# siyi-wind/MDViT

Hardware: AMD Instinct MI355X
Metric: 512x512 images/sec MDViT train step (fwd+bwd, two-sweep, AdamW) (higher is better)
Workload: dtype bf16x3 (fp32 storage; GEMM operands split hi+lo bf16, fp32 accumulate); 1 GPU; MDViT Sup+MLPFM train step, 4 domain(s) x bs=4 per GPU, 512x512, drop_rate=0.1 drop_path=0.1, bf16x3 GEMMs, data-parallel x1

## Files before the change

mdvit_amd/csrc/attn.hip:

```cpp
#include "common.h"
#include "conv_tile.h"

namespace {

constexpr int FA_T = 64;

struct FaGeom {
    int B, H, W, N, C, heads, Ch, s3, s5, s7;
    float scale;
};

typedef float fap_f32x16 __attribute__((ext_vector_type(16)));

template <int CH, bool SOFTMAX>
__global__ __launch_bounds__(256) void fa_partial_kernel(const float* __restrict__ X, long ldx, const float* __restrict__ Y, long ldy,
                                                         const float* __restrict__ ysc, float yscale,
                                                         float* __restrict__ ws_m, float* __restrict__ ws_s, float* __restrict__ ws_P,
                                                         FaGeom g, int NT, int NSUB,
                                                         const float* __restrict__ outp = nullptr, float* __restrict__ dU = nullptr, float* __restrict__ e_part = nullptr) {
    constexpr int GW = CH < 32 ? 32 : CH, NB = (GW + 31) / 32, GQ = GW / 4;
    constexpr int STAGE = 2 * FA_T * GW, RED = 4 * NB * 32 * NB * 32;
    __shared__ __attribute__((aligned(16))) float sm[(STAGE > RED ? STAGE : RED) + 3 * NB * 32 + (SOFTMAX ? 2 * 256 : 0)];
    float* xs = sm;
    float* ys = sm + FA_T * GW;
// ... 394 lines not shown
    }
}

__global__ __launch_bounds__(256) void fa_bwd_prep_kernel(const float* __restrict__ dout, const float* __restrict__ qkv,
                                                          const float* __restrict__ out, const float* __restrict__ a,
                                                          float* __restrict__ dU, float* __restrict__ e, FaGeom g) {
    extern __shared__ float s_e[];
    const int b = blockIdx.y, C = g.C, QC = C >> 2;
    for (int i = threadIdx.x; i < C; i += blockDim.x) s_e[i] = 0.f;
    __syncthreads();
    const long T = (long)gridDim.x * blockDim.x;
    const long t0 = (long)blockIdx.x * blockDim.x + threadIdx.x;
    const int c = (int)(t0 % QC) * 4;
    float4 av = make_float4(1.f, 1.f, 1.f, 1.f);
    if (a) av = *reinterpret_cast<const float4*>(a + (long)b * C + c);
    float4 acc = make_float4(0.f, 0.f, 0.f, 0.f);
    const long total = (long)g.N * QC;
    for (long i = t0; i < total; i += T) {
        const long tok = (long)b * g.N + i / QC;
        const float4 G = *reinterpret_cast<const float4*>(dout + tok * C + c);
        const float4 q = *reinterpret_cast<const float4*>(qkv + tok * 3 * C + c);
        if (dU) *reinterpret_cast<float4*>(dU + tok * C + c) = make_float4(av.x * G.x * q.x, av.y * G.y * q.y, av.z * G.z * q.z, av.w * G.w * q.w);
        if (e) {
            const float4 o = *reinterpret_cast<const float4*>(out + tok * C + c);
            acc.x = fmaf(G.x, o.x, acc.x); acc.y = fmaf(G.y, o.y, acc.y); acc.z = fmaf(G.z, o.z, acc.z); acc.w = fmaf(G.w, o.w, acc.w);
        }
    }
    if (e) {
        atomicAdd(&s_e[c], acc.x); atomicAdd(&s_e[c + 1], acc.y); atomicAdd(&s_e[c + 2], acc.z); atomicAdd(&s_e[c + 3], acc.w);
        __syncthreads();
        for (int i = threadIdx.x; i < C; i += blockDim.x) e[((long)b * gridDim.x + blockIdx.x) * C + i] = s_e[i];
    }
}

typedef float fa_f32x16 __attribute__((ext_vector_type(16)));
template <int CH>
__global__ __launch_bounds__(256) __attribute__((amdgpu_waves_per_eu(2, 2))) void fa_bwd_apply_tab_kernel(const float* __restrict__ dout, const float* __restrict__ qkv,
                                                               const float* __restrict__ U, const float* __restrict__ dVc,
                                                               const float* __restrict__ Mmat, const float* __restrict__ a,
                                                               const float* __restrict__ kmax, const float* __restrict__ ksum,
                                                               const float* __restrict__ dMp, int NTS,
                                                               float* __restrict__ dqkv, FaGeom g, int tokens_per_block) {
    constexpr int C = 8 * CH, C3 = 3 * C, LPT = C / 4, SLOTS = 256 / LPT, LPH = CH / 4, L4 = CH / 4, NS = 8 * L4 + CH;
    __shared__ __attribute__((aligned(16))) float sM[C * CH], sD[C * CH];
    __shared__ __attribute__((aligned(16))) float4 tab[NS][LPT];
    __shared__ float s_tc[C];
    const int b = blockIdx.y;
    for (int i = threadIdx.x; i < C * CH; i += 256) {
        sM[i] = Mmat[(long)b * C * CH + i];
        float dm = 0.f;
        const float* pp = dMp + ((long)b * NTS) * C * CH + i;
        const long rs = (long)C * CH;
        for (int t0 = 0; t0 < NTS; t0 += 8) {
            float v8[8];
#pragma unroll
            for (int u = 0; u < 8; ++u) { const int t = t0 + u; v8[u] = pp[(long)(t < NTS ? t : NTS - 1) * rs]; if (t >= NTS) v8[u] = 0.f; }
#pragma unroll
            for (int u = 0; u < 8; ++u) dm += v8[u];
        }
        sD[i] = dm;
    }
    __syncthreads();
    if (threadIdx.x < C) {
        float tc = 0.f;
#pragma unroll
        for (int e = 0; e < CH; ++e) tc = fmaf(sD[threadIdx.x * CH + e], sM[threadIdx.x * CH + e], tc);
        s_tc[threadIdx.x] = tc;
    }
    for (int i = threadIdx.x; i < NS * LPT; i += 256) {
        const int slot = i / LPT, qq = i % LPT, hl = qq % LPH, hb = (qq / LPH) * CH, cc0 = 4 * qq;
        float4 v;
        if (slot < 8 * L4) {
            const int sl = slot % (4 * L4);
            const float* src = (slot < 4 * L4 ? sM : sD) + (cc0 + sl / L4) * CH + 4 * (hl ^ (sl % L4));
            v = *reinterpret_cast<const float4*>(src);
        } else {
            const int l = slot - 8 * L4, e = 4 * (hl ^ (l >> 2)) + (l & 3);
            v = *reinterpret_cast<const float4*>(sD + (hb + e) * CH + 4 * hl);
        }
        tab[slot][qq] = v;
    }
    __syncthreads();
    const int q = threadIdx.x % LPT, slot = threadIdx.x / LPT;
    const int c0 = 4 * q;
    const long ci = (long)b * C + c0;
    const float4 a4 = a ? *reinterpret_cast<const float4*>(a + ci) : make_float4(1.f, 1.f, 1.f, 1.f);
    const float4 km4 = *reinterpret_cast<const float4*>(kmax + ci);
    float4 is4 = *reinterpret_cast<const float4*>(ksum + ci);
    is4 = make_float4(1.0f / is4.x, 1.0f / is4.y, 1.0f / is4.z, 1.0f / is4.w);
    const float4 tc4 = *reinterpret_cast<const float4*>(s_tc + c0);
    const float inv_scale = 1.0f / g.scale;
    const int n_beg = blockIdx.x * tokens_per_block, n_end = min(g.N, n_beg + tokens_per_block);
    struct Rows { float4 g, k, v, u, c; };
    auto request = [&](Rows& r, int n) __attribute__((always_inline)) {
        const long tok = (long)b * g.N + min(n, g.N - 1);
        r.g = *reinterpret_cast<const float4*>(dout + tok * C + c0);
        r.k = *reinterpret_cast<const float4*>(qkv + tok * C3 + C + c0);
        r.v = *reinterpret_cast<const float4*>(qkv + tok * C3 + 2 * C + c0);
        r.u = *reinterpret_cast<const float4*>(U + tok * C + c0);
        r.c = *reinterpret_cast<const float4*>(dVc + tok * C + c0);
    };
    auto compute = [&](const Rows& r, int n) __attribute__((always_inline)) {
        float dfa[CH], vv[CH], pp[CH];
        dfa[0] = g.scale * a4.x * r.g.x; dfa[1] = g.scale * a4.y * r.g.y; dfa[2] = g.scale * a4.z * r.g.z; dfa[3] = g.scale * a4.w * r.g.w;
        vv[0] = r.v.x; vv[1] = r.v.y; vv[2] = r.v.z; vv[3] = r.v.w;
        pp[0] = expf(r.k.x - km4.x) * is4.x; pp[1] = expf(r.k.y - km4.y) * is4.y; pp[2] = expf(r.k.z - km4.z) * is4.z; pp[3] = expf(r.k.w - km4.w) * is4.w;
#pragma unroll
        for (int j = 0; j < 4; ++j) {
            dfa[4 + j] = fa_dpp_quad_xor<1>(dfa[j]); vv[4 + j] = fa_dpp_quad_xor<1>(vv[j]); pp[4 + j] = fa_dpp_quad_xor<1>(pp[j]);
            if constexpr (CH == 16) {
                dfa[8 + j] = fa_dpp_quad_xor<2>(dfa[j]); dfa[12 + j] = fa_dpp_quad_xor<3>(dfa[j]);
                vv[8 + j] = fa_dpp_quad_xor<2>(vv[j]); vv[12 + j] = fa_dpp_quad_xor<3>(vv[j]);
                pp[8 + j] = fa_dpp_quad_xor<2>(pp[j]); pp[12 + j] = fa_dpp_quad_xor<3>(pp[j]);
            }
        }
        float dq[4], dk[4], dv[4] = {0.f, 0.f, 0.f, 0.f};
        const float uu[4] = {r.u.x, r.u.y, r.u.z, r.u.w}, cc[4] = {r.c.x, r.c.y, r.c.z, r.c.w}, tcv[4] = {tc4.x, tc4.y, tc4.z, tc4.w};
        asm volatile("" ::: "memory");
#pragma unroll
        for (int j = 0; j < 4; ++j) {
            float s1 = 0.f, s2 = 0.f;
#pragma unroll
            for (int l4 = 0; l4 < L4; ++l4) {
                const float4 m4 = tab[L4 * j + l4][q], d4 = tab[4 * L4 + L4 * j + l4][q];
                s1 = fmaf(dfa[4 * l4 + 0], m4.x, s1); s1 = fmaf(dfa[4 * l4 + 1], m4.y, s1); s1 = fmaf(dfa[4 * l4 + 2], m4.z, s1); s1 = fmaf(dfa[4 * l4 + 3], m4.w, s1);
                s2 = fmaf(vv[4 * l4 + 0], d4.x, s2); s2 = fmaf(vv[4 * l4 + 1], d4.y, s2); s2 = fmaf(vv[4 * l4 + 2], d4.z, s2); s2 = fmaf(vv[4 * l4 + 3], d4.w, s2);
            }
            dq[j] = fmaf(dfa[j] * inv_scale, uu[j], s1);
            dk[j] = pp[j] * (s2 - tcv[j]);
        }
#pragma unroll
        for (int l = 0; l < CH; ++l) {
            const float4 dc = tab[8 * L4 + l][q];
            dv[0] = fmaf(pp[l], dc.x, dv[0]); dv[1] = fmaf(pp[l], dc.y, dv[1]); dv[2] = fmaf(pp[l], dc.z, dv[2]); dv[3] = fmaf(pp[l], dc.w, dv[3]);
        }
        if (n < n_end) {
            float* drow = dqkv + ((long)b * g.N + n) * C3 + c0;
            *reinterpret_cast<float4*>(drow) = make_float4(dq[0], dq[1], dq[2], dq[3]);
            *reinterpret_cast<float4*>(drow + C) = make_float4(dk[0], dk[1], dk[2], dk[3]);
            *reinterpret_cast<float4*>(drow + 2 * C) = make_float4(dv[0] + cc[0], dv[1] + cc[1], dv[2] + cc[2], dv[3] + cc[3]);
        }
    };
    Rows ra, rb;
    int n = n_beg + slot;
    request(ra, n);
    for (; n < n_end; n += 2 * SLOTS) {
        request(rb, n + SLOTS);
        compute(ra, n);
        request(ra, n + 2 * SLOTS);
        compute(rb, n + SLOTS);
    }
}

template <int CH, int ROLE>
__device__ __forceinline__ void fa_apply3_tiles(const float* __restrict__ dout, const float* __restrict__ qkv, const float* __restrict__ U, const float* __restrict__ dVc,
                                                float* __restrict__ dqkv, const FaGeom& g, const float* sKV, const float* sD, const float* s_a, const float* s_km,
                                                const float* s_ks, const float* s_tc, int b, int g0, int slot, int tiles_per_block, int bx) {
    constexpr int GW = CH, NB = (GW + 31) / 32, NQ = GW / 8, KS = GW / 2, LD = GW + 1;
    const int C = g.C, C3 = 3 * C;
    const int lane = threadIdx.x & 63;
    const int t = lane & 31, half = lane >> 5;
    const int ntiles = (g.N + 31) / 32;
    const int tile_beg = bx * tiles_per_block, tile_end = min(ntiles, tile_beg + tiles_per_block);
    const float inv_scale = 1.0f / g.scale;
    struct Rows { float4 a[NQ], b[NQ]; };
    auto request = [&](Rows& r, int tile) __attribute__((always_inline)) {
        const long tok = (long)b * g.N + min(tile * 32 + t, g.N - 1);
        const float* arow = ROLE == 0 ? dout + tok * C + g0 : qkv + tok * C3 + C + g0;
        const float* brow = ROLE == 0 ? U + tok * C + g0 : (ROLE == 1 ? qkv + tok * C3 + 2 * C + g0 : dVc + tok * C + g0);
#pragma unroll
        for (int q = 0; q < NQ; ++q) {
            const int cq = 32 * (q / 4) + 8 * (q % 4) + 4 * half;
            r.a[q] = *reinterpret_cast<const float4*>(arow + cq);
            r.b[q] = *reinterpret_cast<const float4*>(brow + cq);
        }
    };
    auto compute = [&](const Rows& r, int tile) __attribute__((always_inline)) {
        const int n = tile * 32 + t;
        const bool ok = n < g.N;
        const float z = ok ? 1.f : 0.f;
        const long tok = (long)b * g.N + (ok ? n : g.N - 1);
        float xo[NQ][4], el[NQ][4];
#pragma unroll
        for (int q = 0; q < NQ; ++q) {
            const int cq = 32 * (q / 4) + 8 * (q % 4) + 4 * half;
            const float4 a4 = r.a[q], b4 = r.b[q];
            if (ROLE == 0) {
                const float4 s4 = *reinterpret_cast<const float4*>(s_a + cq);
                xo[q][0] = z * g.scale * s4.x * a4.x; xo[q][1] = z * g.scale * s4.y * a4.y;
                xo[q][2] = z * g.scale * s4.z * a4.z; xo[q][3] = z * g.scale * s4.w * a4.w;
                el[q][0] = b4.x; el[q][1] = b4.y; el[q][2] = b4.z; el[q][3] = b4.w;
            } else {
                const float4 m4 = *reinterpret_cast<const float4*>(s_km + cq);
                const float4 i4 = *reinterpret_cast<const float4*>(s_ks + cq);
                const float p0 = z * expf(a4.x - m4.x) * i4.x, p1 = z * expf(a4.y - m4.y) * i4.y;
                const float p2 = z * expf(a4.z - m4.z) * i4.z, p3 = z * expf(a4.w - m4.w) * i4.w;
                if (ROLE == 1) {
                    xo[q][0] = z * b4.x; xo[q][1] = z * b4.y; xo[q][2] = z * b4.z; xo[q][3] = z * b4.w;
                    el[q][0] = p0; el[q][1] = p1; el[q][2] = p2; el[q][3] = p3;
                } else {
                    xo[q][0] = p0; xo[q][1] = p1; xo[q][2] = p2; xo[q][3] = p3;
                    el[q][0] = b4.x; el[q][1] = b4.y; el[q][2] = b4.z; el[q][3] = b4.w;
                }
            }
        }
        fa_f32x16 acc[NB];
#pragma unroll
        for (int ob = 0; ob < NB; ++ob)
#pragma unroll
            for (int rr = 0; rr < 16; ++rr) acc[ob][rr] = 0.f;
        asm volatile("" ::: "memory");
#pragma unroll
        for (int ob = 0; ob < NB; ++ob) {
            const int orow = 32 * ob + t;
            const bool rok = orow < GW;
            const int orc = rok ? orow : 0;
#pragma unroll
            for (int kk = 0; kk < KS; ++kk) {
                const int q = kk / 4, j = kk % 4;
                const int kc = 32 * (q / 4) + 8 * (q % 4) + 4 * half + j;
                float w = ROLE == 0 ? sKV[orc * LD + kc] : (ROLE == 1 ? sD[orc * LD + kc] : sD[kc * LD + orc]);
                if (!rok) w = 0.f;
                acc[ob] = __builtin_amdgcn_mfma_f32_32x32x2f32(w, xo[q][j], acc[ob], 0, 0, 0);
            }
        }
        if (ok) {
            float* drow = dqkv + tok * C3 + ROLE * C + g0;
#pragma unroll
            for (int q = 0; q < NQ; ++q) {
                const int ob = q / 4, r0 = 4 * (q % 4);
                const int cq = 32 * (q / 4) + 8 * (q % 4) + 4 * half;
                float4 d;
                if (ROLE == 0) {
                    d.x = fmaf(xo[q][0] * inv_scale, el[q][0], acc[ob][r0 + 0]); d.y = fmaf(xo[q][1] * inv_scale, el[q][1], acc[ob][r0 + 1]);
                    d.z = fmaf(xo[q][2] * inv_scale, el[q][2], acc[ob][r0 + 2]); d.w = fmaf(xo[q][3] * inv_scale, el[q][3], acc[ob][r0 + 3]);
                } else if (ROLE == 1) {
                    const float4 t4 = *reinterpret_cast<const float4*>(s_tc + cq);
                    d.x = el[q][0] * (acc[ob][r0 + 0] - t4.x); d.y = el[q][1] * (acc[ob][r0 + 1] - t4.y);
                    d.z = el[q][2] * (acc[ob][r0 + 2] - t4.z); d.w = el[q][3] * (acc[ob][r0 + 3] - t4.w);
                } else {
                    d.x = acc[ob][r0 + 0] + el[q][0]; d.y = acc[ob][r0 + 1] + el[q][1];
                    d.z = acc[ob][r0 + 2] + el[q][2]; d.w = acc[ob][r0 + 3] + el[q][3];
                }
                *reinterpret_cast<float4*>(drow + cq) = d;
            }
        }
    };
    Rows ra, rb;
    int tile = tile_beg + slot;
    if (tile < tile_end) request(ra, tile);
    for (; tile < tile_end; tile += 4) {
        request(rb, min(tile + 2, ntiles - 1));
        compute(ra, tile);
        if (tile + 2 < tile_end) {
            request(ra, min(tile + 4, ntiles - 1));
            compute(rb, tile + 2);
        }
    }
}

template <int CH>
__global__ __launch_bounds__(384) __attribute__((amdgpu_waves_per_eu(CH >= 64 ? 2 : 3, CH >= 64 ? 2 : 3))) void fa_bwd_apply3_kernel(const float* __restrict__ dout, const float* __restrict__ qkv,
                                                           const float* __restrict__ U, const float* __restrict__ dVc,
                                                           const float* __restrict__ Mmat, const float* __restrict__ a,
                                                           const float* __restrict__ kmax, const float* __restrict__ ksum,
                                                           const float* __restrict__ dMp, int NTS,
                                                           float* __restrict__ dqkv, FaGeom g, int tiles_per_block, int gx, int xcd_map) {
    static_assert(CH >= 32 && CH % 8 == 0, "one head per channel group");
    constexpr int GW = CH, NB = (GW + 31) / 32, NQ = GW / 8, KS = GW / 2, LD = GW + 1, NTH = 384;
    __shared__ float sKV[GW * LD], sD[GW * LD];
    __shared__ __attribute__((aligned(16))) float s_a[GW], s_km[GW], s_ks[GW], s_tc[GW];
    const int C = g.C, C3 = 3 * C;
    int bx, by, bz;
    if (xcd_map) {
        const int nwg = gridDim.x, heads = C / GW;
        const int i = blockIdx.x, slot = (i & 7) * (nwg >> 3) + (i >> 3);
        by = slot % heads; bx = (slot / heads) % gx; bz = slot / (heads * gx);
    } else { bx = blockIdx.x; by = blockIdx.y; bz = blockIdx.z; }
    const int b = bz, g0 = by * GW;
    for (int i = threadIdx.x; i < GW * GW; i += NTH) {
        const int r = i / GW, cc = i % GW;
        sKV[r * LD + cc] = Mmat[((long)b * C + g0 + r) * CH + cc];
        float dm = 0.f;
        const float* pp = dMp + (((long)b * NTS) * C + g0 + r) * CH + cc;
        const long rs = (long)C * CH;
        for (int t0 = 0; t0 < NTS; t0 += 8) {
            float v8[8];
#pragma unroll
            for (int u = 0; u < 8; ++u) { const int t = t0 + u; v8[u] = pp[(long)(t < NTS ? t : NTS - 1) * rs]; if (t >= NTS) v8[u] = 0.f; }
#pragma unroll
            for (int u = 0; u < 8; ++u) dm += v8[u];
        }
        sD[r * LD + cc] = dm;
    }
    for (int i = threadIdx.x; i < GW; i += NTH) {
        const long ci = (long)b * C + g0 + i;
        s_a[i] = a ? a[ci] : 1.f; s_km[i] = kmax[ci]; s_ks[i] = 1.0f / ksum[ci];
    }
    __syncthreads();
    for (int i = threadIdx.x; i < GW; i += NTH) {
        float tc = 0.f;
        for (int e = 0; e < CH; ++e) tc = fmaf(sD[i * LD + e], sKV[i * LD + e], tc);
        s_tc[i] = tc;
    }
    __syncthreads();
    const int wave = threadIdx.x >> 6;
    const int role = wave % 3, slot = wave / 3;
    if (role == 0) fa_apply3_tiles<CH, 0>(dout, qkv, U, dVc, dqkv, g, sKV, sD, s_a, s_km, s_ks, s_tc, b, g0, slot, tiles_per_block, bx);
    else if (role == 1) fa_apply3_tiles<CH, 1>(dout, qkv, U, dVc, dqkv, g, sKV, sD, s_a, s_km, s_ks, s_tc, b, g0, slot, tiles_per_block, bx);
    else fa_apply3_tiles<CH, 2>(dout, qkv, U, dVc, dqkv, g, sKV, sD, s_a, s_km, s_ks, s_tc, b, g0, slot, tiles_per_block, bx);
}

__device__ __forceinline__ void da_fwd_body(float* sm, const float* __restrict__ label, const float* __restrict__ W1, const float* __restrict__ b1,
                                            const float* __restrict__ W2, const float* __restrict__ b2, float* __restrict__ a, int D, int hid, int C, int heads) {
    float* h1 = sm;
    float* z = sm + hid;
    float* zpart = z + C;
    const int b = blockIdx.x, Ch = C / heads, BD = blockDim.x;
    for (int i = threadIdx.x; i < hid; i += BD) {
        float s = 0.f;
        for (int d = 0; d < D; ++d) s = fmaf(label[(long)b * D + d], W1[(long)i * D + d], s);
        h1[i] = fmaxf(s + b1[i], 0.f);
    }
    __syncthreads();
    const bool vec = (hid & 3) == 0 && (reinterpret_cast<uintptr_t>(W2) & 15) == 0;
    const int nq = vec ? hid >> 2 : hid;
    int G = BD / C;
    if (G < 1) G = 1;
    if (G > nq) G = nq;
    for (int c0 = 0; c0 < C; c0 += BD / G) {
        const int c = c0 + (int)threadIdx.x / G, seg = (int)threadIdx.x % G;
        if (c < C && (int)threadIdx.x < (BD / G) * G) {
            const int u0 = (int)((long)nq * seg / G), u1 = (int)((long)nq * (seg + 1) / G);
            const float* wr = W2 + (long)c * hid;
            float s = 0.f;
            if (vec) {
                int u = u0;
                for (; u + 8 <= u1; u += 8) {
                    float4 w4[8];
#pragma unroll
                    for (int q = 0; q < 8; ++q) w4[q] = *reinterpret_cast<const float4*>(wr + 4 * (u + q));
#pragma unroll
                    for (int q = 0; q < 8; ++q) {
                        const int i = 4 * (u + q);
                        s = fmaf(h1[i], w4[q].x, s); s = fmaf(h1[i + 1], w4[q].y, s); s = fmaf(h1[i + 2], w4[q].z, s); s = fmaf(h1[i + 3], w4[q].w, s);
                    }
                }
                for (; u < u1; ++u) {
                    const float4 w4 = *reinterpret_cast<const float4*>(wr + 4 * u);
                    const int i = 4 * u;
                    s = fmaf(h1[i], w4.x, s); s = fmaf(h1[i + 1], w4.y, s); s = fmaf(h1[i + 2], w4.z, s); s = fmaf(h1[i + 3], w4.w, s);
                }
            } else {
                for (int i = u0; i < u1; ++i) s = fmaf(h1[i], wr[i], s);
            }
            zpart[seg * C + c] = s;
        }
    }
    __syncthreads();
    for (int c = threadIdx.x; c < C; c += BD) {
        float s = zpart[c];
        for (int g = 1; g < G; ++g) s += zpart[g * C + c];
        z[c] = s + b2[c];
    }
    __syncthreads();
    for (int c = threadIdx.x; c < C; c += BD) {
        const int ch = c % Ch;
        float m = -INFINITY;
        for (int hh = 0; hh < heads; ++hh) m = fmaxf(m, z[hh * Ch + ch]);
        float s = 0.f;
        for (int hh = 0; hh < heads; ++hh) s += expf(z[hh * Ch + ch] - m);
        a[(long)b * C + c] = expf(z[c] - m) / s;
    }
}
__global__ __launch_bounds__(1024) void da_fwd_kernel(const float* __restrict__ label, const float* __restrict__ W1, const float* __restrict__ b1,
                                                      const float* __restrict__ W2, const float* __restrict__ b2, float* __restrict__ a,
                                                      int D, int hid, int C, int heads) {
    extern __shared__ float sm[];
    da_fwd_body(sm, label, W1, b1, W2, b2, a, D, hid, C, heads);
}
__global__ __launch_bounds__(1024) void da_fwd_many_kernel(MdvitDaMany m, const float* __restrict__ label, int D) {
    extern __shared__ float sm[];
    const int i = blockIdx.y;
    da_fwd_body(sm, label, m.W1[i], m.b1[i], m.W2[i], m.b2[i], m.a[i], D, m.hid[i], m.C[i], m.heads[i]);
}

__device__ __forceinline__ void da_bwd_stage1_body(float* sm, const float* __restrict__ label, const float* __restrict__ W1, const float* __restrict__ b1,
                                                   const float* __restrict__ W2, const float* __restrict__ a, const float* __restrict__ e,
                                                   float* __restrict__ dzbuf, float* __restrict__ hbuf, float* __restrict__ dhbuf,
                                                   int D, int hid, int C, int heads, float scale) {
    float* dz = sm;
    const int b = blockIdx.x, Ch = C / heads;
    for (int c = threadIdx.x; c < C; c += blockDim.x) {
        const int ch = c % Ch;
        float tot = 0.f;
        for (int hh = 0; hh < heads; ++hh) tot += e[(long)b * C + hh * Ch + ch];
        const float v = scale * (e[(long)b * C + c] - a[(long)b * C + c] * tot);
        dz[c] = v;
        dzbuf[(long)b * C + c] = v;
    }
    __syncthreads();
    float* tpart = sm + C;
    const int BD = blockDim.x;
    const int nseg = hid <= BD ? BD / hid : 1;
    for (int i0 = 0; i0 < hid; i0 += BD) {
        const int i = i0 + (int)threadIdx.x % (hid <= BD ? hid : BD), seg = hid <= BD ? (int)threadIdx.x / hid : 0;
        if (i < hid && seg < nseg) {
            const int c_beg = (int)((long)C * seg / nseg), c_end = (int)((long)C * (seg + 1) / nseg);
            float t = 0.f;
#pragma unroll 4
            for (int c = c_beg; c < c_end; ++c) t = fmaf(dz[c], W2[(long)c * hid + i], t);
            tpart[seg * hid + i] = t;
        }
    }
    __syncthreads();
    for (int i = threadIdx.x; i < hid; i += blockDim.x) {
        float s = 0.f;
        for (int d = 0; d < D; ++d) s = fmaf(label[(long)b * D + d], W1[(long)i * D + d], s);
        const float h = s + b1[i];
        float t = 0.f;
        for (int seg = 0; seg < nseg; ++seg) t += tpart[seg * hid + i];
        hbuf[(long)b * hid + i] = fmaxf(h, 0.f);
        dhbuf[(long)b * hid + i] = h > 0.f ? t : 0.f;
    }
}
__global__ __launch_bounds__(1024) void da_bwd_stage1_kernel(const float* __restrict__ label, const float* __restrict__ W1, const float* __restrict__ b1,
                                                            const float* __restrict__ W2, const float* __restrict__ a, const float* __restrict__ e,
                                                            float* __restrict__ dzbuf, float* __restrict__ hbuf, float* __restrict__ dhbuf,
                                                            int D, int hid, int C, int heads, float scale) {
    extern __shared__ float sm[];
    da_bwd_stage1_body(sm, label, W1, b1, W2, a, e, dzbuf, hbuf, dhbuf, D, hid, C, heads, scale);
}
__device__ __forceinline__ void da_bwd_stage2_body(const float* __restrict__ label, const float* __restrict__ dzbuf,
                                                   const float* __restrict__ hbuf, const float* __restrict__ dhbuf,
                                                   float* __restrict__ dW1, float* __restrict__ db1, float* __restrict__ dW2, float* __restrict__ db2,
                                                   int B, int D, int hid, int C) {
    const long i = (long)blockIdx.x * blockDim.x + threadIdx.x;
    const long nW2 = (long)C * hid, nW1 = (long)hid * D;
    if (i < nW2) {
        const int c = (int)(i / hid), j = (int)(i % hid);
        float s = 0.f;
        for (int b = 0; b < B; ++b) s = fmaf(dzbuf[(long)b * C + c], hbuf[(long)b * hid + j], s);
        dW2[i] = s;
    } else if (i < nW2 + nW1) {
        const long k = i - nW2;
        const int j = (int)(k / D), d = (int)(k % D);
        float s = 0.f;
        for (int b = 0; b < B; ++b) s = fmaf(dhbuf[(long)b * hid + j], label[(long)b * D + d], s);
        dW1[k] = s;
    } else if (i < nW2 + nW1 + C) {
        const int c = (int)(i - nW2 - nW1);
        float s = 0.f;
        for (int b = 0; b < B; ++b) s += dzbuf[(long)b * C + c];
        db2[c] = s;
    } else if (i < nW2 + nW1 + C + hid) {
        const int j = (int)(i - nW2 - nW1 - C);
        float s = 0.f;
        for (int b = 0; b < B; ++b) s += dhbuf[(long)b * hid + j];
        db1[j] = s;
    }
}
__global__ __launch_bounds__(256) void da_bwd_stage2_kernel(const float* __restrict__ label, const float* __restrict__ dzbuf,
                                                            const float* __restrict__ hbuf, const float* __restrict__ dhbuf,
                                                            float* __restrict__ dW1, float* __restrict__ db1, float* __restrict__ dW2, float* __restrict__ db2,
                                                            int B, int D, int hid, int C) {
    da_bwd_stage2_body(label, dzbuf, hbuf, dhbuf, dW1, db1, dW2, db2, B, D, hid, C);
}
__device__ __forceinline__ long da_many_ws_offset(const MdvitDaMany& m, int i, int B) {
    long off = 0;
    for (int j = 0; j < i; ++j) off += (long)B * m.C[j] + 2L * B * m.hid[j];
    return off;
}
__global__ __launch_bounds__(1024) void da_bwd_many_stage1_kernel(MdvitDaMany m, MdvitDaManyGrads g, const float* __restrict__ label, float* __restrict__ ws, int B, int D,
                                                                 float scale) {
    extern __shared__ float sm[];
    const int i = blockIdx.y;
    if (!g.e[i]) return;
    float* dzbuf = ws + da_many_ws_offset(m, i, B);
    float* hbuf = dzbuf + (long)B * m.C[i];
    float* dhbuf = hbuf + (long)B * m.hid[i];
    da_bwd_stage1_body(sm, label, m.W1[i], m.b1[i], m.W2[i], m.a[i], g.e[i], dzbuf, hbuf, dhbuf, D, m.hid[i], m.C[i], m.heads[i], scale);
}
__global__ __launch_bounds__(256) void da_bwd_many_stage2_kernel(MdvitDaMany m, MdvitDaManyGrads g, const float* __restrict__ label, const float* __restrict__ ws, int B, int D) {
    const int i = blockIdx.y;
    const int hid = m.hid[i], C = m.C[i];
    if (!g.e[i] || (long)blockIdx.x * blockDim.x >= (long)C * hid + (long)hid * D + C + hid) return;
    const float* dzbuf = ws + da_many_ws_offset(m, i, B);
    const float* hbuf = dzbuf + (long)B * C;
    const float* dhbuf = hbuf + (long)B * hid;
    da_bwd_stage2_body(label, dzbuf, hbuf, dhbuf, g.dW1[i], g.db1[i], g.dW2[i], g.db2[i], B, D, hid, C);
}

bool make_geom(FaGeom& g, int B, int H, int W, int C, int heads, int s3, int s5, int s7) {
    if (B <= 0 || H <= 0 || W <= 0 || C <= 0 || heads <= 0 || C % heads != 0 || C % 4 != 0) return false;
    if (s3 + s5 + s7 != heads) return false;
    g.B = B; g.H = H; g.W = W; g.N = H * W; g.C = C; g.heads = heads; g.Ch = C / heads; g.s3 = s3; g.s5 = s5; g.s7 = s7;
    g.scale = 1.0f / sqrtf((float)g.Ch);
    return true;
}

size_t fa_ws_floats(int B, int N, int C, int heads) {
    const int Ch = C / heads;
    const long NT = (N + FA_T - 1) / FA_T;
    const long fwd = (long)B * NT * C * (2 + Ch);
    const long wg_rows = (long)(cdiv(C, 32) + 2) * B > 1024 ? (long)(cdiv(C, 32) + 2) * B : 1024;
    const long part = wg_rows * 32 * 50 > 1024L * B * C ? wg_rows * 32 * 50 : 1024L * B * C;
    const long bwd = 2L * B * N * C + (long)B * C * (1 + Ch) + (long)B * NT * C * Ch + part;
    return (size_t)(fwd > bwd ? fwd : bwd);
}

int fa_nsub(int NT) { return NT >= 128 ? 8 : (NT >= 64 ? 4 : (NT >= 16 ? 2 : 1)); }

bool fa_built(const FaGeom& g) { return ((g.Ch == 8 || g.Ch == 16) && g.heads == 8) || ((g.Ch == 40 || g.Ch == 64) && g.C <= 512); }
#define FA_CHECK_BUILT(fn, g) MDVIT_CHECK_ARG(fa_built(g), MDVIT_E_SHAPE, fn ": C=%d with %d heads (head dim %d) not built: built are 8 heads at C = 64 / 128 (head dim 8 / 16) " \
                                              "and head dim 40 / 64 with C <= 512 (8 heads at C = 320 / 512)", (g).C, (g).heads, (g).Ch)

int quad_grid(long work_quads, int QC, int max_blocks) {
    int a = QC, b = 256;
    while (b) { int t = a % b; a = b; b = t; }
    const int gmul = QC / a;
    long want = (work_quads + 256L * 4 - 1) / (256L * 4);
    if (want > max_blocks) want = max_blocks;
    if (want < 1) want = 1;
    return (int)((want + gmul - 1) / gmul * gmul);
}

}

extern "C" size_t mdvit_factoratt_ws_bytes(int32_t B, int32_t N, int32_t C, int32_t heads) {
    if (B <= 0 || N <= 0 || C <= 0 || heads <= 0 || C % heads) return 0;
    return fa_ws_floats(B, N, C, heads) * sizeof(float);
}

extern "C" int mdvit_factoratt_fwd(const float* qkv, const float* w3, const float* b3, const float* w5, const float* b5,
                                   const float* w7, const float* b7, const float* a, float* out, float* U, float* kmax, float* ksum, float* Mmat,
                                   void* ws, size_t ws_bytes, int32_t B, int32_t H, int32_t W, int32_t C, int32_t heads,
                                   int32_t s3, int32_t s5, int32_t s7, void* stream) {
    hipStream_t s = (hipStream_t)stream;
    FaGeom g;
    MDVIT_CHECK_ARG(make_geom(g, B, H, W, C, heads, s3, s5, s7), MDVIT_E_SHAPE, "factoratt_fwd: bad geometry B=%d H=%d W=%d C=%d heads=%d splits=%d/%d/%d", B, H, W, C, heads, s3, s5, s7);
    FA_CHECK_BUILT("factoratt_fwd", g);
    MDVIT_CHECK_ARG(ws_bytes >= fa_ws_floats(B, g.N, C, heads) * sizeof(float), MDVIT_E_WORKSPACE, "factoratt_fwd: workspace too small (%zu bytes)", ws_bytes);
    const int Ch = g.Ch, NT0 = cdiv(g.N, FA_T);
    const int NSUB = fa_nsub(NT0);
    const int NT = cdiv(NT0, NSUB);
    float* ws_m = (float*)ws;
    float* ws_s = ws_m + (long)B * NT * C;
    float* ws_P = ws_s + (long)B * NT * C;
#define FA_PART_STREAM(CHV) fa_partial_stream_launch<CHV, true>(dim3(NT, 1, B), s, qkv + C, (long)3 * C, qkv + 2 * C, (long)3 * C, nullptr, 1.f, ws_m, ws_s, ws_P, g, NT0, NSUB, nullptr, nullptr, nullptr)
#define FA_PART_TILES(CHV) hipLaunchKernelGGL((fa_partial_kernel<CHV, true>), dim3(NT, C / CHV, B), dim3(256), 0, s, \
                       qkv + C, (long)3 * C, qkv + 2 * C, (long)3 * C, (const float*)nullptr, 1.f, ws_m, ws_s, ws_P, g, NT0, NSUB)
    switch (Ch) {
        case 8: FA_PART_STREAM(8); break;
        case 16: FA_PART_STREAM(16); break;
        case 40: FA_PART_TILES(40); break;
        case 64: FA_PART_TILES(64); break;
    }
#undef FA_PART_STREAM
#undef FA_PART_TILES
    if (NT > 8)
        hipLaunchKernelGGL((fa_combine_softmax_kernel<32>), dim3(cdiv((long)C * g.Ch, 8), B), dim3(256), 0, s, ws_m, ws_s, ws_P, kmax, ksum, Mmat, g, NT);
    else if (NT > 2)
        hipLaunchKernelGGL((fa_combine_softmax_kernel<4>), dim3(cdiv((long)C * g.Ch, 64), B), dim3(256), 0, s, ws_m, ws_s, ws_P, kmax, ksum, Mmat, g, NT);
    else
        hipLaunchKernelGGL((fa_combine_softmax_kernel<1>), dim3(cdiv((long)C * g.Ch, 256), B), dim3(256), 0, s, ws_m, ws_s, ws_P, kmax, ksum, Mmat, g, NT);
    const int c5 = s3 * Ch, c7 = (s3 + s5) * Ch;
    const CtGeom cg{B, g.H, g.W};
    {
        const int xoff[3] = {2 * C, 2 * C + c5, 2 * C + c7}, yoff[3] = {0, c5, c7}, ncls[3] = {s3 * Ch, s5 * Ch, s7 * Ch};
        const float* const ws3[3] = {w3, w5, w7};
        const float* const bs3[3] = {b3, b5, b7};
        launch_conv3<false>(qkv, 3L * C, xoff, ws3, bs3, U, (long)C, yoff, cg, ncls, s);
    }
    {
        const int TLN = max(1, 256 / C), block = TLN * C;
        int tpb = TLN * 32;
        while (tpb > TLN * 8 && (long)cdiv(g.N, tpb) * B < 1024) tpb /= 2;
        while ((long)cdiv(g.N, tpb) * B > 8192) tpb *= 2;
        dim3 grid(cdiv(g.N, tpb), B);
#define FA_OUT_LAUNCH(CHV) hipLaunchKernelGGL((fa_out_kernel<CHV>), grid, dim3(block), sizeof(float) * FA_OUT_U * TLN * C, s, qkv, U, Mmat, a, out, g, TLN, tpb)
        switch (Ch) {
            case 8: FA_OUT_LAUNCH(8); break;
            case 16: FA_OUT_LAUNCH(16); break;
            case 40: FA_OUT_LAUNCH(40); break;
            case 64: FA_OUT_LAUNCH(64); break;
        }
#undef FA_OUT_LAUNCH
    }
    MDVIT_LAUNCH_CHECK();
    return MDVIT_OK;
}

extern "C" int mdvit_factoratt_bwd(const float* dout, const float* qkv, const float* out, const float* U,
                                   const float* w3, const float* b3, const float* w5, const float* b5, const float* w7, const float* b7,
                                   const float* a, const float* kmax, const float* ksum, const float* Mmat,
                                   float* dqkv, float* e, float* dw3, float* db3, float* dw5, float* db5, float* dw7, float* db7,
                                   void* ws, size_t ws_bytes, int32_t B, int32_t H, int32_t W, int32_t C, int32_t heads,
                                   int32_t s3, int32_t s5, int32_t s7, void* stream) {
    hipStream_t s = (hipStream_t)stream;
    FaGeom g;
    MDVIT_CHECK_ARG(make_geom(g, B, H, W, C, heads, s3, s5, s7), MDVIT_E_SHAPE, "factoratt_bwd: bad geometry B=%d H=%d W=%d C=%d heads=%d", B, H, W, C, heads);
    FA_CHECK_BUILT("factoratt_bwd", g);
    MDVIT_CHECK_ARG(ws_bytes >= fa_ws_floats(B, g.N, C, heads) * sizeof(float), MDVIT_E_WORKSPACE, "factoratt_bwd: workspace too small (%zu bytes)", ws_bytes);
    MDVIT_CHECK_ARG((a == nullptr) == (e == nullptr), MDVIT_E_SHAPE, "factoratt_bwd: a and e must both be given or both be NULL");
    const int Ch = g.Ch, NT = cdiv(g.N, FA_T);
    float* dU = (float*)ws;
    float* dVc = dU + (long)B * g.N * C;
    float* tcol = dVc + (long)B * g.N * C;
    float* dM = tcol + (long)B * C;
    float* ws_P = dM + (long)B * C * Ch;
    const bool want_wgrad = dw3 != nullptr;
    MDVIT_CHECK_ARG(want_wgrad ? (db3 && dw5 && db5 && dw7 && db7) : !(db3 || dw5 || db5 || dw7 || db7), MDVIT_E_SHAPE,
                    "factoratt_bwd: the six crpe gradient outputs must be all given or all NULL");
    if (dqkv == nullptr) {
        MDVIT_CHECK_ARG(e != nullptr && !want_wgrad, MDVIT_E_SHAPE, "factoratt_bwd: dqkv == NULL asks for e alone");
        const int QC0 = C / 4;
        const int gx = quad_grid((long)g.N * QC0, QC0, 512);
        float* e_part = ws_P + (long)B * NT * C * Ch;
        hipLaunchKernelGGL(fa_bwd_prep_kernel, dim3(gx, B), dim3(256), sizeof(float) * C, s, dout, qkv, out, a, (float*)nullptr, e_part, g);
        MDVIT_LAUNCH_CHECK();
        return mdvit_reduce_partials_batched(e_part, B, gx, C, e, s);
    }
    const int NSUBb = fa_nsub(NT), NTS = cdiv(NT, NSUBb);
    float* e_part = ws_P + (long)B * NT * C * Ch;
#define FA_PART_STREAM(CHV) fa_partial_stream_launch<CHV, false>(dim3(NTS, 1, B), s, qkv, (long)3 * C, dout, (long)C, a, g.scale, nullptr, nullptr, ws_P, g, NT, NSUBb, out, dU, e ? e_part : nullptr)
#define FA_PART_TILES(CHV) hipLaunchKernelGGL((fa_partial_kernel<CHV, false>), dim3(NTS, C / CHV, B), dim3(256), 0, s, \
                       qkv, (long)3 * C, dout, (long)C, a, g.scale, (float*)nullptr, (float*)nullptr, ws_P, g, NT, NSUBb, out, dU, e ? e_part : (float*)nullptr)
    switch (Ch) {
        case 8: FA_PART_STREAM(8); break;
        case 16: FA_PART_STREAM(16); break;
        case 40: FA_PART_TILES(40); break;
        case 64: FA_PART_TILES(64); break;
    }
#undef FA_PART_STREAM
#undef FA_PART_TILES
    if (e) {
        const int rc = mdvit_reduce_partials_batched(e_part, B, NTS, C, e, s);
        if (rc != MDVIT_OK) return rc;
    }
    const int c5 = s3 * Ch, c7 = (s3 + s5) * Ch;
    const CtGeom cg{B, g.H, g.W};
    if (want_wgrad) {
        float* wg_part = ws_P + (long)B * NT * C * Ch;
        const int goff[3] = {0, c5, c7}, xoff3[3] = {2 * C, 2 * C + c5, 2 * C + c7}, ncls3[3] = {s3 * Ch, s5 * Ch, s7 * Ch};
        float* const dws[3] = {dw3, dw5, dw7};
        float* const dbs[3] = {db3, db5, db7};
        launch_conv3_wgrad(dU, (long)C, goff, qkv, 3L * C, xoff3, dws, dbs, wg_part, cg, ncls3, s, 0);
    }
    {
        const int off[3] = {0, c5, c7}, ncls[3] = {s3 * Ch, s5 * Ch, s7 * Ch};
        const float* const ws3[3] = {w3, w5, w7};
        launch_conv3<true>(dU, (long)C, off, ws3, nullptr, dVc, (long)C, off, cg, ncls, s);
    }
    if (Ch >= 32) {
        const int ntiles = cdiv(g.N, 32);
        int tpb = 8;
        while (tpb > 2 && (long)cdiv(ntiles, tpb) * heads * B < 256) tpb /= 2;
        const int gx = cdiv(ntiles, tpb);
        const long nwg = (long)gx * heads * B;
        const int xcd_map = nwg % 8 == 0 && nwg < (1L << 30);
        dim3 grid = xcd_map ? dim3((unsigned)nwg, 1, 1) : dim3(gx, heads, B);
        if (Ch == 40) hipLaunchKernelGGL((fa_bwd_apply3_kernel<40>), grid, dim3(384), 0, s, dout, qkv, U, dVc, Mmat, a, kmax, ksum, ws_P, NTS, dqkv, g, tpb, gx, xcd_map);
        else hipLaunchKernelGGL((fa_bwd_apply3_kernel<64>), grid, dim3(384), 0, s, dout, qkv, U, dVc, Mmat, a, kmax, ksum, ws_P, NTS, dqkv, g, tpb, gx, xcd_map);
    } else {
        int tpbk = Ch == 8 ? 1024 : 512;
        while (tpbk > 128 && (long)cdiv(g.N, tpbk) * B < 512) tpbk /= 2;
        const dim3 grid(cdiv(g.N, tpbk), B);
        if (Ch == 8) hipLaunchKernelGGL(fa_bwd_apply_tab_kernel<8>, grid, dim3(256), 0, s, dout, qkv, U, dVc, Mmat, a, kmax, ksum, ws_P, NTS, dqkv, g, tpbk);
        else hipLaunchKernelGGL(fa_bwd_apply_tab_kernel<16>, grid, dim3(256), 0, s, dout, qkv, U, dVc, Mmat, a, kmax, ksum, ws_P, NTS, dqkv, g, tpbk);
    }
    MDVIT_LAUNCH_CHECK();
    return MDVIT_OK;
}

extern "C" int mdvit_factoratt_wgrad(const float* qkv, void* ws, size_t ws_bytes, float* dw3, float* db3, float* dw5, float* db5,
                                     float* dw7, float* db7, int32_t B, int32_t H, int32_t W, int32_t C, int32_t heads,
                                     int32_t s3, int32_t s5, int32_t s7, int32_t accumulate, void* stream) {
    hipStream_t s = (hipStream_t)stream;
    FaGeom g;
    MDVIT_CHECK_ARG(make_geom(g, B, H, W, C, heads, s3, s5, s7), MDVIT_E_SHAPE, "factoratt_wgrad: bad geometry");
    MDVIT_CHECK_ARG(ws_bytes >= fa_ws_floats(B, g.N, C, heads) * sizeof(float), MDVIT_E_WORKSPACE, "factoratt_wgrad: workspace too small");
    MDVIT_CHECK_ARG(dw3 && db3 && dw5 && db5 && dw7 && db7, MDVIT_E_SHAPE, "factoratt_wgrad: all six outputs are required");
    const int Ch = g.Ch, NT = cdiv(g.N, FA_T);
    const float* dU = (const float*)ws;
    float* wg_part = (float*)ws + 2L * B * g.N * C + (long)B * C * (1 + Ch) + (long)B * NT * C * Ch;
    const int c5 = s3 * Ch, c7 = (s3 + s5) * Ch;
    const CtGeom cg{B, g.H, g.W};
    const int goff[3] = {0, c5, c7}, xoff3[3] = {2 * C, 2 * C + c5, 2 * C + c7}, ncls3[3] = {s3 * Ch, s5 * Ch, s7 * Ch};
    float* const dws[3] = {dw3, dw5, dw7};
    float* const dbs[3] = {db3, db5, db7};
    launch_conv3_wgrad(dU, (long)C, goff, qkv, 3L * C, xoff3, dws, dbs, wg_part, cg, ncls3, s, accumulate);
    MDVIT_LAUNCH_CHECK();
    return MDVIT_OK;
}

extern "C" int mdvit_da_fwd(const float* label, const float* W1, const float* b1, const float* W2, const float* b2, float* a,
                            int32_t B, int32_t D, int32_t hid, int32_t C, int32_t heads, void* stream) {
    MDVIT_CHECK_ARG(B > 0 && D > 0 && hid > 0 && C > 0 && heads > 0 && C % heads == 0, MDVIT_E_SHAPE, "da_fwd: bad shape");
    const int G = max(1, min(1024 / C, hid));
    hipLaunchKernelGGL(da_fwd_kernel, dim3(B), dim3(1024), sizeof(float) * (hid + C + (size_t)(G + 1) * C), (hipStream_t)stream, label, W1, b1, W2, b2, a, D, hid, C, heads);
    MDVIT_LAUNCH_CHECK();
    return MDVIT_OK;
}

extern "C" int mdvit_da_fwd_many(const MdvitDaMany* m, const float* label, int32_t B, int32_t D, void* stream) {
    MDVIT_CHECK_ARG(m && label && B > 0 && D > 0 && m->n > 0 && m->n <= MDVIT_DA_MANY_MAX, MDVIT_E_SHAPE, "da_fwd_many: bad arguments");
    size_t smem = 0;
    for (int i = 0; i < m->n; ++i) {
        const int C = m->C[i], hid = m->hid[i];
        MDVIT_CHECK_ARG(m->W1[i] && m->b1[i] && m->W2[i] && m->b2[i] && m->a[i] && hid > 0 && C > 0 && m->heads[i] > 0 && C % m->heads[i] == 0, MDVIT_E_SHAPE,
                        "da_fwd_many: bad adapter %d", i);
        const int G = max(1, min(1024 / C, hid));
        smem = std::max(smem, sizeof(float) * (hid + C + (size_t)(G + 1) * C));
    }
    MDVIT_CHECK_ARG(smem <= 64 * 1024, MDVIT_E_SHAPE, "da_fwd_many: an adapter needs %zu bytes of LDS", smem);
    hipLaunchKernelGGL(da_fwd_many_kernel, dim3(B, m->n), dim3(1024), smem, (hipStream_t)stream, *m, label, D);
    MDVIT_LAUNCH_CHECK();
    return MDVIT_OK;
}

extern "C" size_t mdvit_da_ws_bytes(int32_t B, int32_t hid, int32_t C) {
    if (B <= 0 || hid <= 0 || C <= 0) return 0;
    return sizeof(float) * ((size_t)B * C + 2 * (size_t)B * hid);
}

extern "C" size_t mdvit_da_many_ws_bytes(const MdvitDaMany* m, int32_t B) {
    if (!m || m->n <= 0 || m->n > MDVIT_DA_MANY_MAX || B <= 0) return 0;
    size_t t = 0;
    for (int i = 0; i < m->n; ++i) t += mdvit_da_ws_bytes(B, m->hid[i], m->C[i]);
    return t;
}

extern "C" int mdvit_da_bwd_many(const MdvitDaMany* m, const MdvitDaManyGrads* g, const float* label, float scale, void* ws, size_t ws_bytes, int32_t B, int32_t D,
                                 void* stream) {
    MDVIT_CHECK_ARG(m && g && m->n > 0 && m->n <= MDVIT_DA_MANY_MAX && B > 0 && D > 0, MDVIT_E_SHAPE, "da_bwd_many: bad shape");
    MDVIT_CHECK_ARG(ws_bytes >= mdvit_da_many_ws_bytes(m, B), MDVIT_E_WORKSPACE, "da_bwd_many: workspace too small");
    size_t smem = 0;
    long most = 0;
    bool any = false;
    for (int i = 0; i < m->n; ++i) {
        MDVIT_CHECK_ARG(m->hid[i] > 0 && m->C[i] > 0 && m->heads[i] > 0 && m->C[i] % m->heads[i] == 0, MDVIT_E_SHAPE, "da_bwd_many: bad adapter shape");
        if (!g->e[i]) continue;
        MDVIT_CHECK_ARG(g->dW1[i] && g->db1[i] && g->dW2[i] && g->db2[i], MDVIT_E_SHAPE, "da_bwd_many: an adapter with e needs its four gradient outputs");
        any = true;
        smem = max(smem, sizeof(float) * (m->C[i] + (size_t)max(m->hid[i], 1024)));
        most = max(most, (long)m->C[i] * m->hid[i] + (long)m->hid[i] * D + m->C[i] + m->hid[i]);
    }
    if (!any) return MDVIT_OK;
    hipStream_t s = (hipStream_t)stream;
    hipLaunchKernelGGL(da_bwd_many_stage1_kernel, dim3(B, m->n), dim3(1024), smem, s, *m, *g, label, (float*)ws, B, D, scale);
    hipLaunchKernelGGL(da_bwd_many_stage2_kernel, dim3(cdiv(most, 256), m->n), dim3(256), 0, s, *m, *g, label, (const float*)ws, B, D);
    MDVIT_LAUNCH_CHECK();
    return MDVIT_OK;
}

extern "C" int mdvit_da_bwd(const float* label, const float* W1, const float* b1, const float* W2, const float* b2, const float* a,
                            const float* e, float scale, float* dW1, float* db1, float* dW2, float* db2, void* ws, size_t ws_bytes,
// ... 15 lines not shown
```

Before: 527.1 images/s.

## Coalesce factor-attention apply loads/stores via per-wave LDS transpose staging

Result: no change. 529.1 images/s (median of 6 runs) (+0.4%).

```diff
diff --git a/mdvit_amd/csrc/attn.hip b/mdvit_amd/csrc/attn.hip
--- a/mdvit_amd/csrc/attn.hip
+++ b/mdvit_amd/csrc/attn.hip
@@ -570,56 +570,70 @@
     }
 }
 
+__device__ __forceinline__ void fa_wave_lds_sync() {
+    __builtin_amdgcn_fence(__ATOMIC_RELEASE, "wavefront");
+    __builtin_amdgcn_wave_barrier();
+    __builtin_amdgcn_fence(__ATOMIC_ACQUIRE, "wavefront");
+}
+typedef float fa_f4 __attribute__((ext_vector_type(4)));
 template <int CH, int ROLE>
 __device__ __forceinline__ void fa_apply3_tiles(const float* __restrict__ dout, const float* __restrict__ qkv, const float* __restrict__ U, const float* __restrict__ dVc,
                                                 float* __restrict__ dqkv, const FaGeom& g, const float* sKV, const float* sD, const float* s_a, const float* s_km,
-                                                const float* s_ks, const float* s_tc, int b, int g0, int slot, int tiles_per_block, int bx) {
-    constexpr int GW = CH, NB = (GW + 31) / 32, NQ = GW / 8, KS = GW / 2, LD = GW + 1;
+                                                const float* s_ks, const float* s_tc, float* stg, int b, int g0, int slot, int tiles_per_block, int bx) {
+    constexpr int GW = CH, NB = (GW + 31) / 32, NQ = GW / 8, KS = GW / 2, LD = GW + 1, QR = GW / 4, LDR = GW + 4;
+    static_assert(32 * QR == 64 * NQ && (LDR / 4) % 2 == 1, "NQ wave-wide fa_f4 instructions cover the 32 x GW tile; odd slot stride");
     const int C = g.C, C3 = 3 * C;
     const int lane = threadIdx.x & 63;
     const int t = lane & 31, half = lane >> 5;
     const int ntiles = (g.N + 31) / 32;
     const int tile_beg = bx * tiles_per_block, tile_end = min(ntiles, tile_beg + tiles_per_block);
     const float inv_scale = 1.0f / g.scale;
-    struct Rows { float4 a[NQ], b[NQ]; };
-    auto request = [&](Rows& r, int tile) __attribute__((always_inline)) {
-        const long tok = (long)b * g.N + min(tile * 32 + t, g.N - 1);
-        const float* arow = ROLE == 0 ? dout + tok * C + g0 : qkv + tok * C3 + C + g0;
-        const float* brow = ROLE == 0 ? U + tok * C + g0 : (ROLE == 1 ? qkv + tok * C3 + 2 * C + g0 : dVc + tok * C + g0);
-#pragma unroll
-        for (int q = 0; q < NQ; ++q) {
-            const int cq = 32 * (q / 4) + 8 * (q % 4) + 4 * half;
-            r.a[q] = *reinterpret_cast<const float4*>(arow + cq);
-            r.b[q] = *reinterpret_cast<const float4*>(brow + cq);
+    const float* xbase = (ROLE == 0 ? dout + g0 : (ROLE == 1 ? qkv + 2 * C + g0 : qkv + C + g0)) + (long)b * g.N * (ROLE == 0 ? C : C3);
+    const float* ebase = (ROLE == 0 ? U + g0 : (ROLE == 1 ? qkv + C + g0 : dVc + g0)) + (long)b * g.N * (ROLE == 1 ? C3 : C);
+    float* dbase = dqkv + (long)b * g.N * C3 + ROLE * C + g0;
+    const unsigned ldx = ROLE == 0 ? C : C3, lde = ROLE == 1 ? C3 : C;
+    auto request = [&](fa_f4 (&r)[NQ], const float* base, unsigned ld, int tile) __attribute__((always_inline)) {
+#pragma unroll
+        for (int v = 0; v < NQ; ++v) {
+            const int i = lane + 64 * v, row = i / QR, qd = i % QR;
+            const unsigned tr = (unsigned)min(tile * 32 + row, g.N - 1);
+            r[v] = *reinterpret_cast<const fa_f4*>(reinterpret_cast<const char*>(base) + 4u * (tr * ld + 4u * qd));
         }
     };
-    auto compute = [&](const Rows& r, int tile) __attribute__((always_inline)) {
+    auto transpose = [&](const fa_f4 (&r)[NQ], fa_f4 (&tq)[NQ]) __attribute__((always_inline)) {
+        fa_wave_lds_sync();
+#pragma unroll
+        for (int v = 0; v < NQ; ++v) { const int i = lane + 64 * v; *reinterpret_cast<fa_f4*>(stg + (i / QR) * LDR + 4 * (i % QR)) = r[v]; }
+        fa_wave_lds_sync();
+#pragma unroll
+        for (int q = 0; q < NQ; ++q) tq[q] = *reinterpret_cast<const fa_f4*>(stg + t * LDR + 32 * (q / 4) + 8 * (q % 4) + 4 * half);
+    };
+    auto softmax_p = [&](const fa_f4 k4, int cq, float z, float (&p)[4]) __attribute__((always_inline)) {
+        const fa_f4 m4 = *reinterpret_cast<const fa_f4*>(s_km + cq);
+        const fa_f4 i4 = *reinterpret_cast<const fa_f4*>(s_ks + cq);
+        p[0] = z * expf(k4.x - m4.x) * i4.x; p[1] = z * expf(k4.y - m4.y) * i4.y;
+        p[2] = z * expf(k4.z - m4.z) * i4.z; p[3] = z * expf(k4.w - m4.w) * i4.w;
+    };
+    auto compute = [&](const fa_f4 (&xr)[NQ], int tile) __attribute__((always_inline)) {
         const int n = tile * 32 + t;
         const bool ok = n < g.N;
         const float z = ok ? 1.f : 0.f;
-        const long tok = (long)b * g.N + (ok ? n : g.N - 1);
-        float xo[NQ][4], el[NQ][4];
+        fa_f4 er[NQ], tq[NQ];
+        request(er, ebase, lde, tile);
+        transpose(xr, tq);
+        float xo[NQ][4];
 #pragma unroll
         for (int q = 0; q < NQ; ++q) {
             const int cq = 32 * (q / 4) + 8 * (q % 4) + 4 * half;
-            const float4 a4 = r.a[q], b4 = r.b[q];
+            const fa_f4 x4 = tq[q];
             if (ROLE == 0) {
-                const float4 s4 = *reinterpret_cast<const float4*>(s_a + cq);
-                xo[q][0] = z * g.scale * s4.x * a4.x; xo[q][1] = z * g.scale * s4.y * a4.y;
-                xo[q][2] = z * g.scale * s4.z * a4.z; xo[q][3] = z * g.scale * s4.w * a4.w;
-                el[q][0] = b4.x; el[q][1] = b4.y; el[q][2] = b4.z; el[q][3] = b4.w;
+                const fa_f4 s4 = *reinterpret_cast<const fa_f4*>(s_a + cq);
+                xo[q][0] = z * g.scale * s4.x * x4.x; xo[q][1] = z * g.scale * s4.y * x4.y;
+                xo[q][2] = z * g.scale * s4.z * x4.z; xo[q][3] = z * g.scale * s4.w * x4.w;
+            } else if (ROLE == 1) {
+                xo[q][0] = z * x4.x; xo[q][1] = z * x4.y; xo[q][2] = z * x4.z; xo[q][3] = z * x4.w;
             } else {
-                const float4 m4 = *reinterpret_cast<const float4*>(s_km + cq);
-                const float4 i4 = *reinterpret_cast<const float4*>(s_ks + cq);
-                const float p0 = z * expf(a4.x - m4.x) * i4.x, p1 = z * expf(a4.y - m4.y) * i4.y;
-                const float p2 = z * expf(a4.z - m4.z) * i4.z, p3 = z * expf(a4.w - m4.w) * i4.w;
-                if (ROLE == 1) {
-                    xo[q][0] = z * b4.x; xo[q][1] = z * b4.y; xo[q][2] = z * b4.z; xo[q][3] = z * b4.w;
-                    el[q][0] = p0; el[q][1] = p1; el[q][2] = p2; el[q][3] = p3;
-                } else {
-                    xo[q][0] = p0; xo[q][1] = p1; xo[q][2] = p2; xo[q][3] = p3;
-                    el[q][0] = b4.x; el[q][1] = b4.y; el[q][2] = b4.z; el[q][3] = b4.w;
-                }
+                softmax_p(x4, cq, z, xo[q]);
             }
         }
         fa_f32x16 acc[NB];
@@ -628,52 +642,72 @@
 #pragma unroll
             for (int rr = 0; rr < 16; ++rr) acc[ob][rr] = 0.f;
         asm volatile("" ::: "memory");
-#pragma unroll
-        for (int ob = 0; ob < NB; ++ob) {
+        constexpr int WG = KS % 8 == 0 ? 8 : 10, NG = NB * KS / WG;
+        static_assert(KS % WG == 0, "a group of W elements stays inside one output block");
+        auto wload = [&](float (&w)[WG], int grp) __attribute__((always_inline)) {
+            const int ob = (grp * WG) / KS;
             const int orow = 32 * ob + t;
             const bool rok = orow < GW;
             const int orc = rok ? orow : 0;
 #pragma unroll
-            for (int kk = 0; kk < KS; ++kk) {
-                const int q = kk / 4, j = kk % 4;
+            for (int u = 0; u < WG; ++u) {
+                const int kk = (grp * WG) % KS + u, q = kk / 4, j = kk % 4;
                 const int kc = 32 * (q / 4) + 8 * (q % 4) + 4 * half + j;
-                float w = ROLE == 0 ? sKV[orc * LD + kc] : (ROLE == 1 ? sD[orc * LD + kc] : sD[kc * LD + orc]);
-                if (!rok) w = 0.f;
-                acc[ob] = __builtin_amdgcn_mfma_f32_32x32x2f32(w, xo[q][j], acc[ob], 0, 0, 0);
-            }
-        }
-        if (ok) {
-            float* drow = dqkv + tok * C3 + ROLE * C + g0;
-#pragma unroll
-            for (int q = 0; q < NQ; ++q) {
-                const int ob = q / 4, r0 = 4 * (q % 4);
-                const int cq = 32 * (q / 4) + 8 * (q % 4) + 4 * half;
-                float4 d;
-                if (ROLE == 0) {
-                    d.x = fmaf(xo[q][0] * inv_scale, el[q][0], acc[ob][r0 + 0]); d.y = fmaf(xo[q][1] * inv_scale, el[q][1], acc[ob][r0 + 1]);
-                    d.z = fmaf(xo[q][2] * inv_scale, el[q][2], acc[ob][r0 + 2]); d.w = fmaf(xo[q][3] * inv_scale, el[q][3], acc[ob][r0 + 3]);
-                } else if (ROLE == 1) {
-                    const float4 t4 = *reinterpret_cast<const float4*>(s_tc + cq);
-                    d.x = el[q][0] * (acc[ob][r0 + 0] - t4.x); d.y = el[q][1] * (acc[ob][r0 + 1] - t4.y);
-                    d.z = el[q][2] * (acc[ob][r0 + 2] - t4.z); d.w = el[q][3] * (acc[ob][r0 + 3] - t4.w);
-                } else {
-                    d.x = acc[ob][r0 + 0] + el[q][0]; d.y = acc[ob][r0 + 1] + el[q][1];
-                    d.z = acc[ob][r0 + 2] + el[q][2]; d.w = acc[ob][r0 + 3] + el[q][3];
-                }
-                *reinterpret_cast<float4*>(drow + cq) = d;
-            }
+                const float wv = ROLE == 0 ? sKV[orc * LD + kc] : (ROLE == 1 ? sD[orc * LD + kc] : sD[kc * LD + orc]);
+                w[u] = rok ? wv : 0.f;
+            }
+        };
+#pragma unroll
+        for (int grp = 0; grp < NG; ++grp) {
+            float w[WG];
+            wload(w, grp);
+            const int ob = (grp * WG) / KS;
+#pragma unroll
+            for (int u = 0; u < WG; ++u) {
+                const int kk = (grp * WG) % KS + u, q = kk / 4, j = kk % 4;
+                acc[ob] = __builtin_amdgcn_mfma_f32_32x32x2f32(w[u], xo[q][j], acc[ob], 0, 0, 0);
+            }
+        }
+        transpose(er, tq);
+        fa_wave_lds_sync();
+#pragma unroll
+        for (int q = 0; q < NQ; ++q) {
+            const int ob = q / 4, r0 = 4 * (q % 4);
+            const int cq = 32 * (q / 4) + 8 * (q % 4) + 4 * half;
+            const fa_f4 e4 = tq[q];
+            fa_f4 d;
+            if (ROLE == 0) {
+                d.x = fmaf(xo[q][0] * inv_scale, e4.x, acc[ob][r0 + 0]); d.y = fmaf(xo[q][1] * inv_scale, e4.y, acc[ob][r0 + 1]);
+                d.z = fmaf(xo[q][2] * inv_scale, e4.z, acc[ob][r0 + 2]); d.w = fmaf(xo[q][3] * inv_scale, e4.w, acc[ob][r0 + 3]);
+            } else if (ROLE == 1) {
+                float el[4];
+                softmax_p(e4, cq, z, el);
+                const fa_f4 t4 = *reinterpret_cast<const fa_f4*>(s_tc + cq);
+                d.x = el[0] * (acc[ob][r0 + 0] - t4.x); d.y = el[1] * (acc[ob][r0 + 1] - t4.y);
+                d.z = el[2] * (acc[ob][r0 + 2] - t4.z); d.w = el[3] * (acc[ob][r0 + 3] - t4.w);
+            } else {
+                d.x = acc[ob][r0 + 0] + e4.x; d.y = acc[ob][r0 + 1] + e4.y;
+                d.z = acc[ob][r0 + 2] + e4.z; d.w = acc[ob][r0 + 3] + e4.w;
+            }
+            *reinterpret_cast<fa_f4*>(stg + t * LDR + cq) = d;
+        }
+        fa_wave_lds_sync();
+#pragma unroll
+        for (int v = 0; v < NQ; ++v) {
+            const int i = lane + 64 * v, row = i / QR, qd = i % QR;
+            const int nr = tile * 32 + row;
+            const fa_f4 d = *reinterpret_cast<const fa_f4*>(stg + row * LDR + 4 * qd);
+            if (nr < g.N) *reinterpret_cast<fa_f4*>(reinterpret_cast<char*>(dbase) + 4u * ((unsigned)nr * (unsigned)C3 + 4u * qd)) = d;
         }
     };
-    Rows ra, rb;
+    fa_f4 xa[NQ], xb[NQ];
     int tile = tile_beg + slot;
-    if (tile < tile_end) request(ra, tile);
-    for (; tile < tile_end; tile += 4) {
-        request(rb, min(tile + 2, ntiles - 1));
-        compute(ra, tile);
-        if (tile + 2 < tile_end) {
-            request(ra, min(tile + 4, ntiles - 1));
-            compute(rb, tile + 2);
-        }
+    if (tile < tile_end) request(xa, xbase, ldx, tile);
+    for (; tile < tile_end; tile += 2) {
+        request(xb, xbase, ldx, min(tile + 2, ntiles - 1));
+        compute(xa, tile);
+#pragma unroll
+        for (int v = 0; v < NQ; ++v) xa[v] = xb[v];
     }
 }
 
@@ -685,9 +719,10 @@
                                                            const float* __restrict__ dMp, int NTS,
                                                            float* __restrict__ dqkv, FaGeom g, int tiles_per_block, int gx, int xcd_map) {
     static_assert(CH >= 32 && CH % 8 == 0, "one head per channel group");
-    constexpr int GW = CH, NB = (GW + 31) / 32, NQ = GW / 8, KS = GW / 2, LD = GW + 1, NTH = 384;
+    constexpr int GW = CH, NB = (GW + 31) / 32, NQ = GW / 8, KS = GW / 2, LD = GW + 1, NTH = 384, LDR = GW + 4;
     __shared__ float sKV[GW * LD], sD[GW * LD];
     __shared__ __attribute__((aligned(16))) float s_a[GW], s_km[GW], s_ks[GW], s_tc[GW];
+    __shared__ __attribute__((aligned(16))) float s_stg[(NTH / 64) * 32 * LDR];
     const int C = g.C, C3 = 3 * C;
     int bx, by, bz;
     if (xcd_map) {
@@ -695,6 +730,7 @@
         const int i = blockIdx.x, slot = (i & 7) * (nwg >> 3) + (i >> 3);
         by = slot % heads; bx = (slot / heads) % gx; bz = slot / (heads * gx);
     } else { bx = blockIdx.x; by = blockIdx.y; bz = blockIdx.z; }
+    bx = __builtin_amdgcn_readfirstlane(bx); by = __builtin_amdgcn_readfirstlane(by); bz = __builtin_amdgcn_readfirstlane(bz);
     const int b = bz, g0 = by * GW;
     for (int i = threadIdx.x; i < GW * GW; i += NTH) {
         const int r = i / GW, cc = i % GW;
@@ -724,9 +760,10 @@
     __syncthreads();
     const int wave = threadIdx.x >> 6;
     const int role = wave % 3, slot = wave / 3;
-    if (role == 0) fa_apply3_tiles<CH, 0>(dout, qkv, U, dVc, dqkv, g, sKV, sD, s_a, s_km, s_ks, s_tc, b, g0, slot, tiles_per_block, bx);
-    else if (role == 1) fa_apply3_tiles<CH, 1>(dout, qkv, U, dVc, dqkv, g, sKV, sD, s_a, s_km, s_ks, s_tc, b, g0, slot, tiles_per_block, bx);
-    else fa_apply3_tiles<CH, 2>(dout, qkv, U, dVc, dqkv, g, sKV, sD, s_a, s_km, s_ks, s_tc, b, g0, slot, tiles_per_block, bx);
+    float* stg = s_stg + wave * 32 * LDR;
+    if (role == 0) fa_apply3_tiles<CH, 0>(dout, qkv, U, dVc, dqkv, g, sKV, sD, s_a, s_km, s_ks, s_tc, stg, b, g0, slot, tiles_per_block, bx);
+    else if (role == 1) fa_apply3_tiles<CH, 1>(dout, qkv, U, dVc, dqkv, g, sKV, sD, s_a, s_km, s_ks, s_tc, stg, b, g0, slot, tiles_per_block, bx);
+    else fa_apply3_tiles<CH, 2>(dout, qkv, U, dVc, dqkv, g, sKV, sD, s_a, s_km, s_ks, s_tc, stg, b, g0, slot, tiles_per_block, bx);
 }
 
 __device__ __forceinline__ void da_fwd_body(float* sm, const float* __restrict__ label, const float* __restrict__ W1, const float* __restrict__ b1,
@@ -1021,6 +1058,7 @@
     FA_CHECK_BUILT("factoratt_bwd", g);
     MDVIT_CHECK_ARG(ws_bytes >= fa_ws_floats(B, g.N, C, heads) * sizeof(float), MDVIT_E_WORKSPACE, "factoratt_bwd: workspace too small (%zu bytes)", ws_bytes);
     MDVIT_CHECK_ARG((a == nullptr) == (e == nullptr), MDVIT_E_SHAPE, "factoratt_bwd: a and e must both be given or both be NULL");
+    MDVIT_CHECK_ARG(g.Ch < 32 || (long)g.N * 3 * C * (long)sizeof(float) < (1L << 32), MDVIT_E_SHAPE, "factoratt_bwd: N=%d tokens x C=%d: an image's qkv rows exceed 4 GiB", g.N, C);
     const int Ch = g.Ch, NT = cdiv(g.N, FA_T);
     float* dU = (float*)ws;
     float* dVc = dU + (long)B * g.N * C;
```
